# mborhi/CoMA-UNet

Hardware: AMD Instinct MI355X
Metric: volumes/sec (train fwd+bwd) at 128^3 bf16 (higher is better)
Workload: dtype bf16; 1 GPU; CoMA-UNet train step (fwd + RoiMSE/RnC loss + bwd + all-reduce + AdamW), 128^3 volumes, batch 2/GPU, 6-dim covariates (BASELINE configs[3]); global_batch=2, parallelism=dp1, launch=hipGraph replay of the whole step

## Files before the change

### coma_unet_amd/csrc/conv_mfma.hip

```cpp
#include "common.h"
#include <type_traits>

typedef __attribute__((ext_vector_type(8))) short bf16x8_t;
typedef __attribute__((ext_vector_type(16))) float f32x16_t;

template <typename T> struct elem;
template <> struct elem<bf16_t> { static constexpr int EPB = 8; };
template <> struct elem<float> { static constexpr int EPB = 4; };

__device__ __forceinline__ f32x16_t mma_piece(const uint4& a, const uint4& b, f32x16_t acc, bf16_t) {
  return __builtin_amdgcn_mfma_f32_32x32x16_bf16(*reinterpret_cast<const bf16x8_t*>(&a), *reinterpret_cast<const bf16x8_t*>(&b), acc, 0, 0, 0);
}
__device__ __forceinline__ f32x16_t mma_piece(const uint4& a, const uint4& b, f32x16_t acc, float) {
  acc = __builtin_amdgcn_mfma_f32_32x32x2f32(__uint_as_float(a.x), __uint_as_float(b.x), acc, 0, 0, 0);
  acc = __builtin_amdgcn_mfma_f32_32x32x2f32(__uint_as_float(a.y), __uint_as_float(b.y), acc, 0, 0, 0);
  acc = __builtin_amdgcn_mfma_f32_32x32x2f32(__uint_as_float(a.z), __uint_as_float(b.z), acc, 0, 0, 0);
  acc = __builtin_amdgcn_mfma_f32_32x32x2f32(__uint_as_float(a.w), __uint_as_float(b.w), acc, 0, 0, 0);
  return acc;
}

__device__ __forceinline__ void stat_add(double2* rec, int G, int N, int g, int n, double a, double c) {
  const long rs = ((long)G * N * 2 + 7) & ~7L;
  double* q = reinterpret_cast<double*>(rec) + (long)(blockIdx.x & (COMA_STAT_REPLICAS - 1)) * rs + ((long)g * N + n) * 2;
  unsafeAtomicAdd(q, a);
// ... 2896 lines not shown
      if (FORM == 0) acc[t] = __builtin_amdgcn_mfma_f32_32x32x2f32(d, g[t], acc[t], 0, 0, 0);
      else acc[t] = __builtin_amdgcn_mfma_f32_32x32x2f32(g[t], d, acc[t], 0, 0, 0);
    }
  };

  const int npairs = TM >> 1;
  int tile = tile_begin, tix = 0, tiy = 0, tiz = 0;
  while (tile < tile_end && !tile_coords(tile, p.ntx, p.nty, p.ntz, tix, tiy, tiz)) ++tile;
  if (tile < tile_end) load_next(tix << p.lx, tiy << p.ly, tiz << p.lz);
  while (tile < tile_end) {
    int nt = tile + 1, ntix = 0, ntiy = 0, ntiz = 0;
    while (nt < tile_end && !tile_coords(nt, p.ntx, p.nty, p.ntz, ntix, ntiy, ntiz)) ++nt;
    __syncthreads();
    store_tile();
    __syncthreads();
    if (nt < tile_end) load_next(ntix << p.lx, ntiy << p.ly, ntiz << p.lz);
    float dA, dB, gA[NT], gB[NT];
    rd(ps, dA, gA);
    for (int q = ps; q < npairs; q += 2 * ws) {
      rd(q + ws, dB, gB);
      __builtin_amdgcn_sched_barrier(0);
      mm(dA, gA);
      __builtin_amdgcn_sched_barrier(0);
      rd(q + 2 * ws < npairs ? q + 2 * ws : ps, dA, gA);
      __builtin_amdgcn_sched_barrier(0);
      mm(dB, gB);
      __builtin_amdgcn_sched_barrier(0);
    }
    tile = nt; tix = ntix; tiy = ntiy; tiz = ntiz;
  }
  float* wout = p.dwk + (long)b * p.wsb + (long)(blockIdx.x % (unsigned)p.nrep) * p.rep_stride;
  if constexpr (NT == 7) {
    const int c = c0 + fr;
    const bool full = n0 + 32 <= p.N;
#pragma unroll
    for (int t = 0; t < NT; ++t) {
      const int tap = tg + wt * t;
      if (tap < ntaps && c < p.C) {
        float* pe = wout + ((long)tap * p.N + n0 + 4 * fh) * p.C + c;
#pragma unroll
        for (int e = 0; e < 16; ++e) {
          if (full || n0 + (e & 3) + 8 * (e >> 2) + 4 * fh < p.N) {
            if (p.plain) *pe = acc[t][e]; else atomicAdd(pe, acc[t][e]);
          }
          pe += ((e & 3) == 3 ? 5 : 1) * p.C;
        }
      }
    }
  } else {
#pragma unroll
  for (int t = 0; t < NT; ++t) {
#pragma unroll
    for (int e = 0; e < 16; ++e) {
      const int r = (e & 3) + 8 * (e >> 2) + 4 * fh;
      int tap, n, c;
      if (FORM == 0) {
        const int i = tg + wt * t, tp = i * TPT + (fr >> lcp);
        tap = (i < ntiles && tp < ntaps && gch < chg) ? tp : -1; n = n0 + r; c = c0 + gch;
      } else {
        const int i = tg + wt * t, tp = i * TPT + (r >> lcp), nn = r & (CP - 1);
        tap = (i < ntiles && tp < ntaps && nn < chg) ? tp : -1; n = n0 + nn; c = c0 + fr;
      }
      if (tap >= 0 && n < p.N && c < p.C) {
        if (p.plain) wout[((long)tap * p.N + n) * p.C + c] = acc[t][e];
        else atomicAdd(wout + ((long)tap * p.N + n) * p.C + c, acc[t][e]);
      }
    }
  }
  }
}

struct Wgrad2P {
  const bf16_t* dyp; int ldn; long sbn;
  const bf16_t* xp; int ldc; long sbc;
  int N, C, D, H, W;
  int ntx, nty, ntz, tiles_total, tiles_per_block, cblocks;
  int vec_n, vec_c;
  int lgd, lgg;
  float* dwk; long wsb;
  int nrep; long rep_stride;
};

template <int HX, int HY, int NT>
__device__ __forceinline__ void wgrad2_tile(const char* Dt, const char* Gt, int lane_d, int lane_g, const int (&toff)[NT],
                                            int ntap, f32x16_t (&acc)[NT], int ks0, int ksd) {
  constexpr int PD = 64, PG = 64;
  auto rd_d = [&](int ks) -> bf16x8_t {
    const int z = ks >> 3, y = (ks >> 1) & 3, xh = ks & 1;
    const char* dp = Dt + lane_d + ((z * 4 + y) * 32 + xh * 16) * PD;
    const s4_t dlo = __builtin_amdgcn_ds_read_tr16_b64_v4i16((lds_s4_t*)(dp));
    const s4_t dhi = __builtin_amdgcn_ds_read_tr16_b64_v4i16((lds_s4_t*)(dp + 4 * PD));
    return (bf16x8_t){dlo[0], dlo[1], dlo[2], dlo[3], dhi[0], dhi[1], dhi[2], dhi[3]};
  };
  auto rd_g = [&](int ks, int t) -> bf16x8_t {
    const int z = ks >> 3, y = (ks >> 1) & 3, xh = ks & 1;
    const char* gp = Gt + lane_g + ((z * HY + y) * HX + xh * 16) * PG;
    const s4_t glo = __builtin_amdgcn_ds_read_tr16_b64_v4i16((lds_s4_t*)(gp + toff[t]));
    const s4_t ghi = __builtin_amdgcn_ds_read_tr16_b64_v4i16((lds_s4_t*)(gp + toff[t] + 4 * PG));
    return (bf16x8_t){glo[0], glo[1], glo[2], glo[3], ghi[0], ghi[1], ghi[2], ghi[3]};
  };
  (void)ntap;
  bf16x8_t df = rd_d(ks0), gf = rd_g(ks0, 0);
#pragma unroll 2
  for (int ks = ks0; ks < 16; ks += ksd) {
    const int kn = ks + ksd < 16 ? ks + ksd : ks;
    bf16x8_t dn = df;
#pragma unroll
    for (int t = 0; t < NT; ++t) {
      bf16x8_t gn;
      if (t + 1 < NT) gn = rd_g(ks, t + 1);
      else { dn = rd_d(kn); gn = rd_g(kn, 0); }
      __builtin_amdgcn_sched_barrier(0);
      acc[t] = __builtin_amdgcn_mfma_f32_32x32x16_bf16(df, gf, acc[t], 0, 0, 0);
      __builtin_amdgcn_sched_barrier(0);
      gf = gn;
    }
    df = dn;
  }
}

template <int VEC, int OCC, int K, int PK>
__global__ __launch_bounds__(256, OCC) void conv_mfma_wgrad2_k(Wgrad2P p) {
  constexpr int PADK = (K - 1) / 2;
  constexpr int NTILE = K == 1 ? 1 : (PK == 1 ? 27 : PK == 2 ? 18 : 9), NT = (NTILE + 3) / 4;
  constexpr int TX = 32, TY = 4, TZ = 2, TM = TX * TY * TZ, HX = TX + K - 1, HY = TY + K - 1, HZ = TZ + K - 1, HV = HX * HY * HZ;
  constexpr int NDP = TM * 4, NGP = HV * 4;
  constexpr int DIT = NDP / 256, GIT = (NGP + 255) / 256;
  extern __shared__ __attribute__((aligned(16))) char smem[];
  char* Dt = smem;
  char* Gt = smem + TM * 64;
  const int tid = threadIdx.x, lane = tid & 63;
  const int wid = __builtin_amdgcn_readfirstlane(tid >> 6);
  const int b = blockIdx.z;
  const int nb = blockIdx.y / p.cblocks, cb = blockIdx.y % p.cblocks;
  const int n0 = nb * 32, c0 = cb * 32;
  const bf16_t* dyb = p.dyp + (long)b * p.sbn + n0;
  const bf16_t* xb = p.xp + (long)b * p.sbc + c0;
  const int chn = p.N - n0, chc = p.C - c0;
  const int lgd = PK == 1 ? 2 : p.lgd, lgg = PK == 1 ? 2 : p.lgg;
  const int chd = tid & ((1 << lgd) - 1), chg = tid & ((1 << lgg) - 1);
  const bool dlive = chd * 8 < chn, glive = chg * 8 < chc;

  for (int i = tid; i < NDP + NGP; i += 256) reinterpret_cast<uint4*>(smem)[i] = make_uint4(0, 0, 0, 0);

  f32x16_t acc[NT];
#pragma unroll
  for (int t = 0; t < NT; ++t)
#pragma unroll
    for (int e = 0; e < 16; ++e) acc[t][e] = 0.f;

  const int g16 = lane >> 4, li = lane & 15, q = li >> 2, pp = li & 3;
  const int vrow = 8 * (g16 >> 1) + q;
  const int chan_b = ((g16 & 1) * 16 + 4 * pp) * 2;
  const int lane_d = vrow * 64 + chan_b;
  const int chunk = (g16 & 1) * 4 + pp;
  const int lane_g = PK == 1 ? vrow * 64 + chan_b
                   : PK == 2 ? (vrow + (chunk >> 2)) * 64 + (chunk & 3) * 8
                             : (vrow + (chunk >> 1)) * 64 + (chunk & 1) * 8;

  int toff[NT];
#pragma unroll
  for (int t = 0; t < NT; ++t) {
    const int i = wid + 4 * t < NTILE ? wid + 4 * t : 0;
    const int row = PK == 1 ? i / 3 : PK == 2 ? i >> 1 : i, kx0 = PK == 1 ? i % 3 : PK == 2 ? (i & 1) * 2 : 0;
    toff[t] = K == 1 ? 0 : __builtin_amdgcn_readfirstlane((((row / 3) * HY + row % 3) * HX + kx0) * 64);
  }
  const int ntap = K == 1 ? 1 : (NTILE - wid + 3) / 4;

  const int tile_begin = xcd_remap(blockIdx.x, gridDim.x) * p.tiles_per_block;
  int tile_end = tile_begin + p.tiles_per_block;
  if (tile_end > p.tiles_total) tile_end = p.tiles_total;

  uint4 dv[DIT], gv[GIT];
  auto load_tile = [&](int x0, int y0, int z0) {
    if (dlive) {
#pragma unroll
      for (int it = 0; it < DIT; ++it) {
        const int row = (tid + 256 * it) >> lgd;
        const int vx = row & 31, vy = (row >> 5) & 3, vz = row >> 7;
        const int gz = z0 + vz, gy = y0 + vy, gx = x0 + vx;
        dv[it] = make_uint4(0, 0, 0, 0);
        if (row < TM && gz < p.D && gy < p.H && gx < p.W) {
          const bf16_t* src = dyb + (unsigned)(((gz * p.H + gy) * p.W + gx) * p.ldn + chd * 8);
          dv[it] = VEC ? *reinterpret_cast<const uint4*>(src) : load8_raw(src, chn - chd * 8, p.vec_n);
        }
      }
    }
    if (glive) {
#pragma unroll
      for (int it = 0; it < GIT; ++it) {
        const int row = (tid + 256 * it) >> lgg;
        const int hx = row % HX, hy = (row / HX) % HY, hz = row / (HX * HY);
        const int gz = z0 - PADK + hz, gy = y0 - PADK + hy, gx = x0 - PADK + hx;
        gv[it] = make_uint4(0, 0, 0, 0);
        if (row < HV && (unsigned)gz < (unsigned)p.D && (unsigned)gy < (unsigned)p.H && (unsigned)gx < (unsigned)p.W) {
          const bf16_t* src = xb + (unsigned)(((gz * p.H + gy) * p.W + gx) * p.ldc + chg * 8);
          gv[it] = VEC ? *reinterpret_cast<const uint4*>(src) : load8_raw(src, chc - chg * 8, p.vec_c);
        }
      }
    }
  };
  const uint4 dmask = mask8(VEC ? 8 : chn - chd * 8), gmask = mask8(VEC ? 8 : chc - chg * 8);
  auto and4 = [](uint4 v, uint4 m) { v.x &= m.x; v.y &= m.y; v.z &= m.z; v.w &= m.w; return v; };
  auto store_tile = [&]() {
    if (dlive) {
#pragma unroll
      for (int it = 0; it < DIT; ++it) {
        const int row = (tid + 256 * it) >> lgd;
        if (row < TM) reinterpret_cast<uint4*>(Dt)[row * 4 + chd] = VEC ? dv[it] : and4(dv[it], dmask);
      }
    }
    if (glive) {
#pragma unroll
      for (int it = 0; it < GIT; ++it) {
        const int row = (tid + 256 * it) >> lgg;
        if (row < HV) reinterpret_cast<uint4*>(Gt)[row * 4 + chg] = VEC ? gv[it] : and4(gv[it], gmask);
      }
    }
  };

  int tile = tile_begin, tix = 0, tiy = 0, tiz = 0;
  while (tile < tile_end && !tile_coords(tile, p.ntx, p.nty, p.ntz, tix, tiy, tiz)) ++tile;
  if (tile < tile_end) load_tile(tix * TX, tiy * TY, tiz * TZ);
  while (tile < tile_end) {
    int nt = tile + 1, ntix = 0, ntiy = 0, ntiz = 0;
    while (nt < tile_end && !tile_coords(nt, p.ntx, p.nty, p.ntz, ntix, ntiy, ntiz)) ++nt;
    __syncthreads();
    store_tile();
    __syncthreads();
    constexpr bool EARLY = OCC == 1 || PK > 1 || K == 1;
    if (EARLY) { if (nt < tile_end) load_tile(ntix * TX, ntiy * TY, ntiz * TZ); }
    wgrad2_tile<HX, HY, NT>(Dt, Gt, lane_d, lane_g, toff, ntap, acc, K == 1 ? wid : 0, K == 1 ? 4 : 1);
    if (!EARLY) { if (nt < tile_end) load_tile(ntix * TX, ntiy * TY, ntiz * TZ); }
    tile = nt;
  }
  float* wout = p.dwk + (long)b * p.wsb + (long)(blockIdx.x % (unsigned)p.nrep) * p.rep_stride;
  const int fr = lane & 31, fh = lane >> 5;
  const int sub = PK == 1 ? 0 : PK == 2 ? fr >> 4 : fr >> 3;
  const int cc = PK == 1 ? fr : PK == 2 ? (fr & 15) : (fr & 7);
#pragma unroll
  for (int t = 0; t < NT; ++t) {
    const int i = wid + 4 * t;
    const int row = PK == 1 ? i / 3 : PK == 2 ? i >> 1 : i, kx = (PK == 1 ? i % 3 : PK == 2 ? (i & 1) * 2 : 0) + sub;
    const int tap = K == 1 ? 0 : row * 3 + kx;
    if (t < ntap && kx < 3) {
#pragma unroll
      for (int e = 0; e < 16; ++e) {
        const int n = n0 + (e & 3) + 8 * (e >> 2) + 4 * fh;
        const int c = c0 + cc;
        if (n < p.N && c < p.C) atomicAdd(wout + ((long)tap * p.N + n) * p.C + c, acc[t][e]);
      }
    }
  }
}

static bool wgrad2_ok(const coma_conv_desc* d, const coma_tensor* x, const coma_tensor* dy) {
  return d->form == 0 && d->stride == 1 && (d->ksize == 3 || d->ksize == 1) && x->dtype == COMA_BF16 && dy->dtype == COMA_BF16 &&
         x->W >= 32 && (long)t_vox(x) * x->ld < (1L << 31) && (long)t_vox(dy) * dy->ld < (1L << 31);
}

#define WGRAD_NREP 64
#define WGRAD_REP_MAX_ELEMS 16384
static long wgrad_out_elems(const coma_conv_desc* d, const coma_tensor* x, const coma_tensor* dy) {
  return (long)d->ksize * d->ksize * d->ksize * dy->C * x->C * (d->per_sample_w ? x->B : 1);
}
__global__ __launch_bounds__(256) void wgrad_replica_sum_k(const float* __restrict__ rep, int nrep, long n, float* __restrict__ out) {
  const long i = (long)blockIdx.x * 32 + (threadIdx.x >> 3);
  const int part = threadIdx.x & 7;
  float a = 0.f;
  if (i < n) {
#pragma unroll 8
    for (int r = part; r < nrep; r += 8) a += rep[(long)r * n + i];
  }
  a += __shfl_xor(a, 4, 64); a += __shfl_xor(a, 2, 64); a += __shfl_xor(a, 1, 64);
  if (part == 0 && i < n) out[i] = a;
}

struct Thin16FWP {
  const float* x; int ldx; long sbx; int D, H, W, C;
  const float* dy; int ldn; long sbn; int N;
  unsigned xbytes, dbytes;
  int ntx, nty, ntz, ids_total, ids_per_block;
  float* dwk; long wsb;
  int nrep; long rep_stride;
};

template <int CP, int NB>
__global__ __launch_bounds__(256, CP == 16 ? 1 : 2) void conv_thin16f_wgrad_k(Thin16FWP p) {
  constexpr int TX = 32, TY = 4, TZ = 2, HX = TX + 2, HY = TY + 2, HZ = TZ + 2, HV = HX * HY * HZ, TM = TX * TY * TZ;
  constexpr int TPM = 16 / CP, NM = (27 + TPM - 1) / TPM;
  constexpr int ND = NB * 16;
  constexpr int PCH = CP / 4, DCH = ND / 4;
  constexpr int HP = HV * PCH, DP = TM * DCH, HIT = (HP + 255) / 256, DIT = DP / 256, NIT = HIT + DIT;
  static_assert(NIT <= 32, "two staging pieces per K step at most");
  extern __shared__ __attribute__((aligned(16))) char smem[];
  float* Hl = reinterpret_cast<float*>(smem);
  float* Dl = Hl + HV * CP;
  const int tid = threadIdx.x, lane = tid & 63;
  const int wid = __builtin_amdgcn_readfirstlane(tid >> 6);
  const int b = blockIdx.z;
  const int lv = lane & 15, lg = lane >> 4;
  const float* xb = p.x + (long)b * p.sbx;
  const float* db = p.dy + (long)b * p.sbn;
  const __amdgpu_buffer_rsrc_t rs_x = __builtin_amdgcn_make_buffer_rsrc(const_cast<float*>(xb), 0, p.xbytes, 0x00020000);
  const __amdgpu_buffer_rsrc_t rs_d = __builtin_amdgcn_make_buffer_rsrc(const_cast<float*>(db), 0, p.dbytes, 0x00020000);
  constexpr unsigned OOB = 0x7fff0000u;

  int s_z[NIT], s_y[NIT], s_x[NIT];
  unsigned s_boff[NIT];
#pragma unroll
  for (int it = 0; it < NIT; ++it) {
    if (it < HIT) {
      const int piece = tid + 256 * it;
      const int row = piece / PCH, ch = piece % PCH;
      const int hx = row % HX, hy = (row / HX) % HY, hz = row / (HX * HY);
      s_z[it] = piece < HP ? hz - 1 : (1 << 20); s_y[it] = hy - 1; s_x[it] = hx - 1;
      s_boff[it] = (unsigned)(ch * 16);
// ... 666 lines not shown
  q.wsb = d->per_sample_w ? wsz1 : 0;
  q.dwk = dwk;
  if (!(zeroed & COMA_ZEROED_OUT) && hipMemsetAsync(dwk, 0, sizeof(float) * wsz, s) != hipSuccess) { coma_set_error("wgrad memset failed"); return 2; }
  const size_t lds = S == 1 ? (size_t)(34 * 6 * 4 + 256) * 64 : (size_t)(65 * 5 * 3 + 64) * 64;
  static bool attr = false;
  if (!attr) {
    (void)hipFuncSetAttribute((const void*)conv_bf16_wgrad16_k<1, 0>, hipFuncAttributeMaxDynamicSharedMemorySize, 80 * 1024);
    (void)hipFuncSetAttribute((const void*)conv_bf16_wgrad16_k<2, 0>, hipFuncAttributeMaxDynamicSharedMemorySize, 80 * 1024);
    (void)hipFuncSetAttribute((const void*)conv_bf16_wgrad16_k<2, 1>, hipFuncAttributeMaxDynamicSharedMemorySize, 80 * 1024);
    attr = true;
  }
  const dim3 grid((unsigned)gx, (unsigned)pairs, (unsigned)x->B);
  coma_set_kernel_tag("conv_bf16_wgrad16_k<%d, %d>", S, d->form);
  if (S == 1) hipLaunchKernelGGL((conv_bf16_wgrad16_k<1, 0>), grid, dim3(256), lds, s, q);
  else if (d->form == 0) hipLaunchKernelGGL((conv_bf16_wgrad16_k<2, 0>), grid, dim3(256), lds, s, q);
  else hipLaunchKernelGGL((conv_bf16_wgrad16_k<2, 1>), grid, dim3(256), lds, s, q);
  COMA_LAUNCH_CHECK();
  return 0;
}

static bool thin16f_wgrad_ok(const coma_conv_desc* d, const coma_tensor* x, const coma_tensor* dy) {
  static const bool on = []{ const char* e = getenv("COMA_THIN16F"); return !(e && e[0] == '0'); }();
  const int nmax = x->C <= 4 ? 32 : 16;
  return on && d->form == 0 && d->ksize == 3 && d->stride == 1 && x->dtype == COMA_F32 && dy->dtype == COMA_F32 && x->W >= 32 &&
         x->C <= 16 && dy->C <= nmax && x->ld % 4 == 0 && x->sb % 4 == 0 && dy->ld % 4 == 0 && dy->sb % 4 == 0 &&
         (!x->data || aligned16(x->data)) && (!dy->data || aligned16(dy->data)) &&
         (unsigned long long)t_vox(x) * x->ld * 4 < 0x7fff0000ull && (unsigned long long)t_vox(dy) * dy->ld * 4 < 0x7fff0000ull;
}

static int conv_thin16f_wgrad(const coma_conv_desc* d, const coma_tensor* x, const coma_tensor* dy, float* dwk, void* ws,
                              size_t ws_bytes, hipStream_t s, int zeroed) {
  Thin16FWP q;
  q.x = (const float*)x->data; q.ldx = (int)x->ld; q.sbx = x->sb; q.D = x->D; q.H = x->H; q.W = x->W; q.C = x->C;
  q.dy = (const float*)dy->data; q.ldn = (int)dy->ld; q.sbn = dy->sb; q.N = dy->C;
  q.xbytes = (unsigned)((unsigned long long)t_vox(x) * x->ld * 4);
  q.dbytes = (unsigned)((unsigned long long)t_vox(dy) * dy->ld * 4);
  q.ntx = (q.W + 31) / 32; q.nty = (q.H + 3) / 4; q.ntz = (q.D + 1) / 2;
  q.ids_total = q.ntx * q.nty * ((q.ntz + 7) / 8) * 8;
  int gx = (q.C > 8 ? 256 : 512) / x->B;
  if (gx < 1) gx = 1;
  if (gx > q.ids_total) gx = q.ids_total;
  q.ids_per_block = (q.ids_total + gx - 1) / gx;
  gx = (q.ids_total + q.ids_per_block - 1) / q.ids_per_block;
  const long wsz1 = 27L * q.N * q.C, wsz = wsz1 * (d->per_sample_w ? x->B : 1);
  q.wsb = d->per_sample_w ? wsz1 : 0;
  const bool replicas = wsz <= WGRAD_REP_MAX_ELEMS && ws && ws_bytes >= sizeof(float) * wsz * WGRAD_NREP;
  q.nrep = replicas ? WGRAD_NREP : 1;
  q.rep_stride = replicas ? wsz : 0;
  q.dwk = replicas ? (float*)ws : dwk;
  if (!(zeroed & (replicas ? COMA_ZEROED_WS : COMA_ZEROED_OUT)) && hipMemsetAsync(q.dwk, 0, sizeof(float) * wsz * q.nrep, s) != hipSuccess) { coma_set_error("wgrad memset failed"); return 2; }
  const int cp = q.C > 8 ? 16 : q.C > 4 ? 8 : 4, nb = q.N > 16 ? 2 : 1;
  const int nm = (27 + 16 / cp - 1) / (16 / cp);
  size_t lds = (size_t)34 * 6 * 4 * cp * 4 + (size_t)256 * nb * 16 * 4;
  if (lds < (size_t)nm * nb * 256 * 4) lds = (size_t)nm * nb * 256 * 4;
  static bool attr = false;
  if (!attr) {
    (void)hipFuncSetAttribute((const void*)conv_thin16f_wgrad_k<16, 1>, hipFuncAttributeMaxDynamicSharedMemorySize, 80 * 1024);
    (void)hipFuncSetAttribute((const void*)conv_thin16f_wgrad_k<8, 1>, hipFuncAttributeMaxDynamicSharedMemorySize, 80 * 1024);
    (void)hipFuncSetAttribute((const void*)conv_thin16f_wgrad_k<4, 1>, hipFuncAttributeMaxDynamicSharedMemorySize, 80 * 1024);
    (void)hipFuncSetAttribute((const void*)conv_thin16f_wgrad_k<4, 2>, hipFuncAttributeMaxDynamicSharedMemorySize, 80 * 1024);
    attr = true;
  }
  const dim3 grid((unsigned)gx, 1, (unsigned)x->B);
  coma_set_kernel_tag("conv_thin16f_wgrad_k<%d, %d>", cp, nb);
  if (cp == 16) hipLaunchKernelGGL((conv_thin16f_wgrad_k<16, 1>), grid, dim3(256), lds, s, q);
  else if (cp == 8) hipLaunchKernelGGL((conv_thin16f_wgrad_k<8, 1>), grid, dim3(256), lds, s, q);
  else if (nb == 2) hipLaunchKernelGGL((conv_thin16f_wgrad_k<4, 2>), grid, dim3(256), lds, s, q);
  else hipLaunchKernelGGL((conv_thin16f_wgrad_k<4, 1>), grid, dim3(256), lds, s, q);
  COMA_LAUNCH_CHECK();
  if (replicas) {
    hipLaunchKernelGGL(wgrad_replica_sum_k, dim3((unsigned)((wsz + 31) / 32)), dim3(256), 0, s, (const float*)ws, WGRAD_NREP, wsz, dwk);
    COMA_LAUNCH_CHECK();
  }
  return 0;
}

static int conv_mfma_wgrad2(const coma_conv_desc* d, const coma_tensor* x, const coma_tensor* dy, float* dwk, void* ws,
                            size_t ws_bytes, hipStream_t s, int zeroed) {
  Wgrad2P p;
  p.dyp = (const bf16_t*)dy->data; p.ldn = (int)dy->ld; p.sbn = dy->sb;
  p.xp = (const bf16_t*)x->data; p.ldc = (int)x->ld; p.sbc = x->sb;
  p.N = dy->C; p.C = x->C; p.D = x->D; p.H = x->H; p.W = x->W;
  p.ntx = (p.W + 31) / 32; p.nty = (p.H + 3) / 4; p.ntz = (p.D + 1) / 2;
  p.tiles_total = p.ntx * p.nty * ((p.ntz + 7) / 8) * 8;
  p.cblocks = (p.C + 31) / 32;
  {
    const int nd = p.N > 32 ? 4 : (p.N + 7) / 8, ng = p.C > 32 ? 4 : (p.C + 7) / 8;
    p.lgd = nd <= 1 ? 0 : nd <= 2 ? 1 : 2; p.lgg = ng <= 1 ? 0 : ng <= 2 ? 1 : 2;
  }
  const int pairs = ((p.N + 31) / 32) * p.cblocks;
  p.vec_n = dy->ld % 8 == 0 && dy->sb % 8 == 0 && (((uintptr_t)dy->data) & 15) == 0;
  p.vec_c = x->ld % 8 == 0 && x->sb % 8 == 0 && (((uintptr_t)x->data) & 15) == 0;
  int chunks = 512 / (pairs * x->B);
  if (chunks < 1) chunks = 1;
  if (chunks > p.tiles_total) chunks = p.tiles_total;
  p.tiles_per_block = (p.tiles_total + chunks - 1) / chunks;
  chunks = (p.tiles_total + p.tiles_per_block - 1) / p.tiles_per_block;
  const long taps = (long)d->ksize * d->ksize * d->ksize;
  p.dwk = dwk; p.wsb = d->per_sample_w ? taps * p.N * p.C : 0;
  const long wsz = taps * p.N * p.C * (d->per_sample_w ? x->B : 1);
  const bool replicas = wsz <= WGRAD_REP_MAX_ELEMS && ws && ws_bytes >= sizeof(float) * wsz * WGRAD_NREP;
  p.nrep = replicas ? WGRAD_NREP : 1;
  p.rep_stride = replicas ? wsz : 0;
  if (replicas) p.dwk = (float*)ws;
  if (!(zeroed & (replicas ? COMA_ZEROED_WS : COMA_ZEROED_OUT)) && hipMemsetAsync(p.dwk, 0, sizeof(float) * wsz * p.nrep, s) != hipSuccess) { coma_set_error("wgrad memset failed"); return 2; }
  const size_t lds = (size_t)(256 + (d->ksize == 3 ? 816 + 1 : 256)) * 64;
  static bool attr = false;
  if (!attr) {
    (void)hipFuncSetAttribute((const void*)conv_mfma_wgrad2_k<0, 2, 3, 1>, hipFuncAttributeMaxDynamicSharedMemorySize, 80 * 1024);
    (void)hipFuncSetAttribute((const void*)conv_mfma_wgrad2_k<1, 2, 3, 1>, hipFuncAttributeMaxDynamicSharedMemorySize, 80 * 1024);
    (void)hipFuncSetAttribute((const void*)conv_mfma_wgrad2_k<0, 2, 3, 2>, hipFuncAttributeMaxDynamicSharedMemorySize, 80 * 1024);
    (void)hipFuncSetAttribute((const void*)conv_mfma_wgrad2_k<1, 2, 3, 2>, hipFuncAttributeMaxDynamicSharedMemorySize, 80 * 1024);
    (void)hipFuncSetAttribute((const void*)conv_mfma_wgrad2_k<0, 2, 3, 4>, hipFuncAttributeMaxDynamicSharedMemorySize, 80 * 1024);
    (void)hipFuncSetAttribute((const void*)conv_mfma_wgrad2_k<1, 2, 3, 4>, hipFuncAttributeMaxDynamicSharedMemorySize, 80 * 1024);
    attr = true;
  }
  const bool vec = p.vec_n && p.vec_c && p.N % 8 == 0 && p.C % 8 == 0;
  const dim3 grid((unsigned)chunks, (unsigned)pairs, (unsigned)x->B);
  coma_set_kernel_tag("conv_mfma_wgrad2_k<%d, 2, %d, %d>", (int)vec, d->ksize, d->ksize == 1 ? 1 : p.C <= 8 ? 4 : p.C <= 16 ? 2 : 1);
#define WG2(K_, PK_) do { if (vec) hipLaunchKernelGGL((conv_mfma_wgrad2_k<1, 2, K_, PK_>), grid, dim3(256), lds, s, p); \
                          else hipLaunchKernelGGL((conv_mfma_wgrad2_k<0, 2, K_, PK_>), grid, dim3(256), lds, s, p); } while (0)
  if (d->ksize == 1) WG2(1, 1);
  else if (p.C <= 8) WG2(3, 4);
  else if (p.C <= 16) WG2(3, 2);
  else WG2(3, 1);
#undef WG2
  COMA_LAUNCH_CHECK();
  if (replicas) {
    hipLaunchKernelGGL(wgrad_replica_sum_k, dim3((unsigned)((wsz + 31) / 32)), dim3(256), 0, s, (const float*)ws, WGRAD_NREP, wsz, dwk);
    COMA_LAUNCH_CHECK();
  }
  return 0;
}

static int ilog2_ceil(int v) { int l = 0; while ((1 << l) < v) ++l; return l; }

struct WgradPlan { WgradP2 p; int TM; size_t lds; int tn, tc; dim3 grid; bool ok; };

static WgradPlan wgrad_plan(const coma_conv_desc* d, const coma_tensor* x, const coma_tensor* dy) {
  WgradPlan pl{};
  pl.ok = false;
  const bool f32 = x->dtype == COMA_F32 && dy->dtype == COMA_F32;
  if (!f32 && (x->dtype != COMA_BF16 || dy->dtype != COMA_BF16)) return pl;
  if (d->ksize != 3 && d->ksize != 1) return pl;
  if ((long)t_vox(x) * x->ld >= (1L << 31) || (long)t_vox(dy) * dy->ld >= (1L << 31)) return pl;
  if (d->form == 1 && d->stride != 2) return pl;
  WgradP2& p = pl.p;
  p.dyp = dy->data; p.ldn = (int)dy->ld; p.sbn = dy->sb;
  p.xp = x->data; p.ldc = (int)x->ld; p.sbc = x->sb;
  p.N = dy->C; p.C = x->C;
  const coma_tensor* dn = d->form == 0 ? dy : x;
  const coma_tensor* ga = d->form == 0 ? x : dy;
  p.Mz = dn->D; p.My = dn->H; p.Mx = dn->W; p.Gz = ga->D; p.Gy = ga->H; p.Gx = ga->W;
  p.k = d->ksize; p.stride = d->stride; p.pad = d->pad;
  const int vq = f32 ? 4 : 8;
  p.vec_n = dy->ld % vq == 0 && dy->sb % vq == 0 && (!dy->data || aligned16(dy->data));
  p.vec_c = x->ld % vq == 0 && x->sb % vq == 0 && (!x->data || aligned16(x->data));
  pl.tn = (dy->C > 32 && !(x->C > 32 && x->C > dy->C)) ? 2 : 1;
  pl.tc = (pl.tn == 1 && x->C > 32) ? 2 : 1;
  if (f32) pl.tn = pl.tc = 1;
  const int gch = d->form == 0 ? x->C : dy->C;
  const int esz = f32 ? 4 : 2, ppc = f32 ? 4 : 8, maxp = f32 ? ((gch >= 32 && d->ksize == 3) ? 21 : 24) : 20;
  p.cp = 32; p.pg = 128;
  if (f32 && gch < 32) { p.cp = 1; while (p.cp < gch) p.cp <<= 1; p.pg = (p.cp < 4 ? 4 : p.cp) * 4; }
  if (f32 && !(p.vec_n && p.vec_c)) return pl;
  const int cdb = 32 * (d->form == 0 ? pl.tn : pl.tc), cgb = f32 ? p.pg / 4 : 32 * (d->form == 0 ? pl.tc : pl.tn);
  bool fits = false;
  for (int budget = d->stride == 1 ? 8 : 6; budget >= 4 && !fits; --budget) {
    int lx = ilog2_ceil(p.Mx); if (lx > 5) lx = 5;
    if (d->stride == 2 && lx > 4) lx = 4;
    if (lx > budget) lx = budget;
    int rem = budget - lx;
    int ly = ilog2_ceil(p.My); if (ly > (rem + 1) / 2) ly = (rem + 1) / 2;
    rem -= ly;
    int lz = ilog2_ceil(p.Mz); if (lz > rem) lz = rem;
    while (lx + ly + lz < 4) ++lx;
    p.lx = lx; p.ly = ly; p.lz = lz;
    pl.TM = 1 << (lx + ly + lz);
    p.hz = ((1 << lz) - 1) * p.stride + p.k; p.hy = ((1 << ly) - 1) * p.stride + p.k; p.hx = ((1 << lx) - 1) * p.stride + p.k;
    pl.lds = (size_t)pl.TM * cdb * esz + (size_t)p.hz * p.hy * p.hx * cgb * esz + (f32 ? 1024 : 0);
    fits = pl.lds <= 160 * 1024 && pl.TM * (cdb / ppc) + p.hz * p.hy * p.hx * (cgb / ppc) <= 256 * maxp;
  }
  if (!fits) return pl;
  p.ntx = (p.Mx + (1 << p.lx) - 1) >> p.lx; p.nty = (p.My + (1 << p.ly) - 1) >> p.ly; p.ntz = (p.Mz + (1 << p.lz) - 1) >> p.lz;
  p.tiles_total = p.ntx * p.nty * ((p.ntz + 7) / 8) * 8;
  p.m_hx = (unsigned)((1ull << 32) / (unsigned)p.hx) + 1u;
  p.m_hxy = (unsigned)((1ull << 32) / (unsigned)(p.hx * p.hy)) + 1u;
  p.cblocks = (p.C + 32 * pl.tc - 1) / (32 * pl.tc);
  const int pairs = ((p.N + 32 * pl.tn - 1) / (32 * pl.tn)) * p.cblocks;
  int chunks = 256 / (pairs * x->B);
  if (pairs * x->B >= 64 && (long)p.Mz * p.My * p.Mx <= 1024) chunks = 1;
  if (chunks < 1) chunks = 1;
  if (chunks > p.tiles_total) chunks = p.tiles_total;
  p.tiles_per_block = (p.tiles_total + chunks - 1) / chunks;
  chunks = (p.tiles_total + p.tiles_per_block - 1) / p.tiles_per_block;
  p.plain = chunks == 1 && (d->per_sample_w || x->B == 1);
  if (f32 && p.cp < 8 && d->ksize == 3) p.plain = 0;
  if (f32 && d->ksize == 1) p.plain = 0;
  pl.grid = dim3((unsigned)chunks, (unsigned)pairs, (unsigned)x->B);
  const long taps = (long)d->ksize * d->ksize * d->ksize;
  p.wsb = d->per_sample_w ? taps * p.N * p.C : 0;
  pl.ok = true;
  return pl;
}
// ... 76 lines not shown
```

Baseline: 118.7 volumes/s.

## Ping-pong two warp groups in 3x3x3 wgrad kernel to overlap loads with MFMA

For the K=3, PK=1 weight-gradient kernel, the block grows to 512 threads split into two 256-thread groups, each with its own LDS tile buffer. The groups alternate between staging a tile (global load plus LDS store) and computing MFMA on it, synchronized with duo_barrier, so memory traffic of one group overlaps compute of the other. The two groups' partial accumulators are reduced through LDS before the atomic write-out, and the grid halves its chunk count to compensate. The non-group path now always issues the next tile load early. The cost is double LDS per block (up to 160KB), occupancy 1, and an extra cross-group reduction.

After: 119.3 volumes/s, median of 6. About the same (+0.5%).

```diff
diff --git a/coma_unet_amd/csrc/conv_mfma.hip b/coma_unet_amd/csrc/conv_mfma.hip
--- a/coma_unet_amd/csrc/conv_mfma.hip
+++ b/coma_unet_amd/csrc/conv_mfma.hip
@@ -3040,17 +3040,20 @@
 }
 
 template <int VEC, int OCC, int K, int PK>
-__global__ __launch_bounds__(256, OCC) void conv_mfma_wgrad2_k(Wgrad2P p) {
+__global__ __launch_bounds__(K == 3 && PK == 1 ? 512 : 256, K == 3 && PK == 1 ? 1 : OCC) void conv_mfma_wgrad2_k(Wgrad2P p) {
+  constexpr bool GROUPS = K == 3 && PK == 1;
   constexpr int PADK = (K - 1) / 2;
   constexpr int NTILE = K == 1 ? 1 : (PK == 1 ? 27 : PK == 2 ? 18 : 9), NT = (NTILE + 3) / 4;
   constexpr int TX = 32, TY = 4, TZ = 2, TM = TX * TY * TZ, HX = TX + K - 1, HY = TY + K - 1, HZ = TZ + K - 1, HV = HX * HY * HZ;
   constexpr int NDP = TM * 4, NGP = HV * 4;
   constexpr int DIT = NDP / 256, GIT = (NGP + 255) / 256;
+  constexpr int IMG = (TM + HV + 1) * 64;
   extern __shared__ __attribute__((aligned(16))) char smem[];
-  char* Dt = smem;
-  char* Gt = smem + TM * 64;
-  const int tid = threadIdx.x, lane = tid & 63;
-  const int wid = __builtin_amdgcn_readfirstlane(tid >> 6);
+  const int wall = __builtin_amdgcn_readfirstlane(threadIdx.x >> 6);
+  const int grp = GROUPS ? wall >> 2 : 0, wid = wall & 3;
+  const int tid = threadIdx.x & 255, lane = tid & 63;
+  char* Dt = smem + grp * IMG;
+  char* Gt = Dt + TM * 64;
   const int b = blockIdx.z;
   const int nb = blockIdx.y / p.cblocks, cb = blockIdx.y % p.cblocks;
   const int n0 = nb * 32, c0 = cb * 32;
@@ -3061,7 +3064,7 @@
   const int chd = tid & ((1 << lgd) - 1), chg = tid & ((1 << lgg) - 1);
   const bool dlive = chd * 8 < chn, glive = chg * 8 < chc;
 
-  for (int i = tid; i < NDP + NGP; i += 256) reinterpret_cast<uint4*>(smem)[i] = make_uint4(0, 0, 0, 0);
+  for (int i = tid; i < NDP + NGP; i += 256) reinterpret_cast<uint4*>(Dt)[i] = make_uint4(0, 0, 0, 0);
 
   f32x16_t acc[NT];
 #pragma unroll
@@ -3139,6 +3142,60 @@
     }
   };
 
+  if constexpr (GROUPS) {
+    const int nsteps = (tile_end - tile_begin + 1) / 2;
+    auto tile_of = [&](int s, int& x0, int& y0, int& z0) -> bool {
+      const int id = tile_begin + 2 * s + grp;
+      int tx = 0, ty = 0, tz = 0;
+      const bool ok = id < tile_end && tile_coords(id, p.ntx, p.nty, p.ntz, tx, ty, tz);
+      x0 = tx * TX; y0 = ty * TY; z0 = tz * TZ;
+      return __builtin_amdgcn_readfirstlane((int)ok) != 0;
+    };
+    auto stage = [&](int s) __attribute__((always_inline)) {
+      int x0, y0, z0;
+      if (tile_of(s, x0, y0, z0)) { load_tile(x0, y0, z0); store_tile(); }
+    };
+    auto compute = [&](int s) __attribute__((always_inline)) {
+      int x0, y0, z0;
+      if (tile_of(s, x0, y0, z0)) wgrad2_tile<HX, HY, NT>(Dt, Gt, lane_d, lane_g, toff, ntap, acc, 0, 1);
+    };
+    __syncthreads();
+    if (grp == 0) {
+      stage(0);
+      duo_barrier();
+#pragma unroll 1
+      for (int s = 0; s < nsteps; ++s) {
+        compute(s); duo_barrier();
+        stage(s + 1); duo_barrier();
+      }
+    } else {
+      duo_barrier();
+#pragma unroll 1
+      for (int s = 0; s < nsteps; ++s) {
+        stage(s); duo_barrier();
+        compute(s); duo_barrier();
+      }
+    }
+    __syncthreads();
+    f32x4_t* xa = reinterpret_cast<f32x4_t*>(smem) + wid * (NT * 4 * 64) + lane;
+    if (grp == 1) {
+#pragma unroll
+      for (int t = 0; t < NT; ++t)
+#pragma unroll
+        for (int j = 0; j < 4; ++j)
+          xa[(t * 4 + j) * 64] = (f32x4_t){acc[t][4 * j], acc[t][4 * j + 1], acc[t][4 * j + 2], acc[t][4 * j + 3]};
+    }
+    __syncthreads();
+    if (grp == 1) return;
+#pragma unroll
+    for (int t = 0; t < NT; ++t)
+#pragma unroll
+      for (int j = 0; j < 4; ++j) {
+        const f32x4_t v = xa[(t * 4 + j) * 64];
+#pragma unroll
+        for (int e = 0; e < 4; ++e) acc[t][4 * j + e] += v[e];
+      }
+  } else {
   int tile = tile_begin, tix = 0, tiy = 0, tiz = 0;
   while (tile < tile_end && !tile_coords(tile, p.ntx, p.nty, p.ntz, tix, tiy, tiz)) ++tile;
   if (tile < tile_end) load_tile(tix * TX, tiy * TY, tiz * TZ);
@@ -3148,11 +3205,10 @@
     __syncthreads();
     store_tile();
     __syncthreads();
-    constexpr bool EARLY = OCC == 1 || PK > 1 || K == 1;
-    if (EARLY) { if (nt < tile_end) load_tile(ntix * TX, ntiy * TY, ntiz * TZ); }
+    if (nt < tile_end) load_tile(ntix * TX, ntiy * TY, ntiz * TZ);
     wgrad2_tile<HX, HY, NT>(Dt, Gt, lane_d, lane_g, toff, ntap, acc, K == 1 ? wid : 0, K == 1 ? 4 : 1);
-    if (!EARLY) { if (nt < tile_end) load_tile(ntix * TX, ntiy * TY, ntiz * TZ); }
     tile = nt;
+  }
   }
   float* wout = p.dwk + (long)b * p.wsb + (long)(blockIdx.x % (unsigned)p.nrep) * p.rep_stride;
   const int fr = lane & 31, fh = lane >> 5;
@@ -3994,7 +4050,8 @@
   const int pairs = ((p.N + 31) / 32) * p.cblocks;
   p.vec_n = dy->ld % 8 == 0 && dy->sb % 8 == 0 && (((uintptr_t)dy->data) & 15) == 0;
   p.vec_c = x->ld % 8 == 0 && x->sb % 8 == 0 && (((uintptr_t)x->data) & 15) == 0;
-  int chunks = 512 / (pairs * x->B);
+  const bool groups = d->ksize == 3 && p.C > 16;
+  int chunks = (groups ? 256 : 512) / (pairs * x->B);
   if (chunks < 1) chunks = 1;
   if (chunks > p.tiles_total) chunks = p.tiles_total;
   p.tiles_per_block = (p.tiles_total + chunks - 1) / chunks;
@@ -4007,11 +4064,11 @@
   p.rep_stride = replicas ? wsz : 0;
   if (replicas) p.dwk = (float*)ws;
   if (!(zeroed & (replicas ? COMA_ZEROED_WS : COMA_ZEROED_OUT)) && hipMemsetAsync(p.dwk, 0, sizeof(float) * wsz * p.nrep, s) != hipSuccess) { coma_set_error("wgrad memset failed"); return 2; }
-  const size_t lds = (size_t)(256 + (d->ksize == 3 ? 816 + 1 : 256)) * 64;
+  const size_t lds = (size_t)(256 + (d->ksize == 3 ? 816 + 1 : 256)) * 64 * (groups ? 2 : 1);
   static bool attr = false;
   if (!attr) {
-    (void)hipFuncSetAttribute((const void*)conv_mfma_wgrad2_k<0, 2, 3, 1>, hipFuncAttributeMaxDynamicSharedMemorySize, 80 * 1024);
-    (void)hipFuncSetAttribute((const void*)conv_mfma_wgrad2_k<1, 2, 3, 1>, hipFuncAttributeMaxDynamicSharedMemorySize, 80 * 1024);
+    (void)hipFuncSetAttribute((const void*)conv_mfma_wgrad2_k<0, 2, 3, 1>, hipFuncAttributeMaxDynamicSharedMemorySize, 160 * 1024);
+    (void)hipFuncSetAttribute((const void*)conv_mfma_wgrad2_k<1, 2, 3, 1>, hipFuncAttributeMaxDynamicSharedMemorySize, 160 * 1024);
     (void)hipFuncSetAttribute((const void*)conv_mfma_wgrad2_k<0, 2, 3, 2>, hipFuncAttributeMaxDynamicSharedMemorySize, 80 * 1024);
     (void)hipFuncSetAttribute((const void*)conv_mfma_wgrad2_k<1, 2, 3, 2>, hipFuncAttributeMaxDynamicSharedMemorySize, 80 * 1024);
     (void)hipFuncSetAttribute((const void*)conv_mfma_wgrad2_k<0, 2, 3, 4>, hipFuncAttributeMaxDynamicSharedMemorySize, 80 * 1024);
@@ -4021,8 +4078,9 @@
   const bool vec = p.vec_n && p.vec_c && p.N % 8 == 0 && p.C % 8 == 0;
   const dim3 grid((unsigned)chunks, (unsigned)pairs, (unsigned)x->B);
   coma_set_kernel_tag("conv_mfma_wgrad2_k<%d, 2, %d, %d>", (int)vec, d->ksize, d->ksize == 1 ? 1 : p.C <= 8 ? 4 : p.C <= 16 ? 2 : 1);
-#define WG2(K_, PK_) do { if (vec) hipLaunchKernelGGL((conv_mfma_wgrad2_k<1, 2, K_, PK_>), grid, dim3(256), lds, s, p); \
-                          else hipLaunchKernelGGL((conv_mfma_wgrad2_k<0, 2, K_, PK_>), grid, dim3(256), lds, s, p); } while (0)
+  const dim3 block(groups ? 512 : 256);
+#define WG2(K_, PK_) do { if (vec) hipLaunchKernelGGL((conv_mfma_wgrad2_k<1, 2, K_, PK_>), grid, block, lds, s, p); \
+                          else hipLaunchKernelGGL((conv_mfma_wgrad2_k<0, 2, K_, PK_>), grid, block, lds, s, p); } while (0)
   if (d->ksize == 1) WG2(1, 1);
   else if (p.C <= 8) WG2(3, 4);
   else if (p.C <= 16) WG2(3, 2);
```

## Reuse halo z-planes across consecutive tiles in 3x3x3 wgrad via LDS ring

Applied to the files above, without the earlier changes.

For 3x3x3 weight-gradient convolutions, tiles are now walked z-first within each (x,y) column, and the input halo is kept in a 4-plane LDS ring. Each new tile loads only the TZ new z-planes instead of the full HZ-plane halo, and only the first tile of a column loads the full halo. Per-tap LDS offsets are recomputed each tile from the ring position. This cuts global input traffic and LDS stores, but makes tile ordering column-major, so load-balancing and the locality of blocks across XCDs change. The early/late prefetch choice is also removed, so the next tile is always prefetched before compute.

After: 118.7 volumes/s before, 119.4 volumes/s after, median of 6. No clear change (+0.6%).

```diff
diff --git a/coma_unet_amd/csrc/conv_mfma.hip b/coma_unet_amd/csrc/conv_mfma.hip
--- a/coma_unet_amd/csrc/conv_mfma.hip
+++ b/coma_unet_amd/csrc/conv_mfma.hip
@@ -3002,8 +3002,8 @@
 };
 
 template <int HX, int HY, int NT>
-__device__ __forceinline__ void wgrad2_tile(const char* Dt, const char* Gt, int lane_d, int lane_g, const int (&toff)[NT],
-                                            int ntap, f32x16_t (&acc)[NT], int ks0, int ksd) {
+__device__ __forceinline__ void wgrad2_tile(const char* Dt, const char* Gt, int lane_d, int lane_g, const int (&toff0)[NT],
+                                            const int (&toff1)[NT], int ntap, f32x16_t (&acc)[NT], int ks0, int ksd) {
   constexpr int PD = 64, PG = 64;
   auto rd_d = [&](int ks) -> bf16x8_t {
     const int z = ks >> 3, y = (ks >> 1) & 3, xh = ks & 1;
@@ -3015,8 +3015,9 @@
   auto rd_g = [&](int ks, int t) -> bf16x8_t {
     const int z = ks >> 3, y = (ks >> 1) & 3, xh = ks & 1;
     const char* gp = Gt + lane_g + ((z * HY + y) * HX + xh * 16) * PG;
-    const s4_t glo = __builtin_amdgcn_ds_read_tr16_b64_v4i16((lds_s4_t*)(gp + toff[t]));
-    const s4_t ghi = __builtin_amdgcn_ds_read_tr16_b64_v4i16((lds_s4_t*)(gp + toff[t] + 4 * PG));
+    const int to = z ? toff1[t] : toff0[t];
+    const s4_t glo = __builtin_amdgcn_ds_read_tr16_b64_v4i16((lds_s4_t*)(gp + to));
+    const s4_t ghi = __builtin_amdgcn_ds_read_tr16_b64_v4i16((lds_s4_t*)(gp + to + 4 * PG));
     return (bf16x8_t){glo[0], glo[1], glo[2], glo[3], ghi[0], ghi[1], ghi[2], ghi[3]};
   };
   (void)ntap;
@@ -3039,12 +3040,23 @@
   }
 }
 
+__device__ __forceinline__ bool wgrad2_tile_coords(int id, int nty, int ntz, int& tix, int& tiy, int& tiz) {
+  const int col = id / ntz;
+  tiz = id - col * ntz;
+  tix = col / nty;
+  tiy = col - tix * nty;
+  return true;
+}
+
 template <int VEC, int OCC, int K, int PK>
 __global__ __launch_bounds__(256, OCC) void conv_mfma_wgrad2_k(Wgrad2P p) {
   constexpr int PADK = (K - 1) / 2;
   constexpr int NTILE = K == 1 ? 1 : (PK == 1 ? 27 : PK == 2 ? 18 : 9), NT = (NTILE + 3) / 4;
   constexpr int TX = 32, TY = 4, TZ = 2, TM = TX * TY * TZ, HX = TX + K - 1, HY = TY + K - 1, HZ = TZ + K - 1, HV = HX * HY * HZ;
-  constexpr int NDP = TM * 4, NGP = HV * 4;
+  constexpr bool RING = K == 3;
+  constexpr int PLR = HX * HY, PLB = PLR * 64;
+  constexpr int GROWS = RING ? TZ * PLR : HV;
+  constexpr int NDP = TM * 4, NGP = GROWS * 4;
   constexpr int DIT = NDP / 256, GIT = (NGP + 255) / 256;
   extern __shared__ __attribute__((aligned(16))) char smem[];
   char* Dt = smem;
@@ -3061,7 +3073,7 @@
   const int chd = tid & ((1 << lgd) - 1), chg = tid & ((1 << lgg) - 1);
   const bool dlive = chd * 8 < chn, glive = chg * 8 < chc;
 
-  for (int i = tid; i < NDP + NGP; i += 256) reinterpret_cast<uint4*>(smem)[i] = make_uint4(0, 0, 0, 0);
+  for (int i = tid; i < (TM + HV) * 4; i += 256) reinterpret_cast<uint4*>(smem)[i] = make_uint4(0, 0, 0, 0);
 
   f32x16_t acc[NT];
 #pragma unroll
@@ -3078,21 +3090,25 @@
                    : PK == 2 ? (vrow + (chunk >> 2)) * 64 + (chunk & 3) * 8
                              : (vrow + (chunk >> 1)) * 64 + (chunk & 1) * 8;
 
-  int toff[NT];
+  int tkz[NT], trow[NT];
 #pragma unroll
   for (int t = 0; t < NT; ++t) {
     const int i = wid + 4 * t < NTILE ? wid + 4 * t : 0;
     const int row = PK == 1 ? i / 3 : PK == 2 ? i >> 1 : i, kx0 = PK == 1 ? i % 3 : PK == 2 ? (i & 1) * 2 : 0;
-    toff[t] = K == 1 ? 0 : __builtin_amdgcn_readfirstlane((((row / 3) * HY + row % 3) * HX + kx0) * 64);
+    tkz[t] = K == 1 ? 0 : row / 3;
+    trow[t] = K == 1 ? 0 : ((row % 3) * HX + kx0) * 64;
   }
   const int ntap = K == 1 ? 1 : (NTILE - wid + 3) / 4;
 
   const int tile_begin = xcd_remap(blockIdx.x, gridDim.x) * p.tiles_per_block;
   int tile_end = tile_begin + p.tiles_per_block;
   if (tile_end > p.tiles_total) tile_end = p.tiles_total;
+  auto coords = [&](int id, int& tix, int& tiy, int& tiz) {
+    return RING ? wgrad2_tile_coords(id, p.nty, p.ntz, tix, tiy, tiz) : tile_coords(id, p.ntx, p.nty, p.ntz, tix, tiy, tiz);
+  };
 
   uint4 dv[DIT], gv[GIT];
-  auto load_tile = [&](int x0, int y0, int z0) {
+  auto load_d = [&](int x0, int y0, int z0) __attribute__((always_inline)) {
     if (dlive) {
 #pragma unroll
       for (int it = 0; it < DIT; ++it) {
@@ -3106,14 +3122,16 @@
         }
       }
     }
+  };
+  auto load_g = [&](int x0, int y0, int zp) __attribute__((always_inline)) {
     if (glive) {
 #pragma unroll
       for (int it = 0; it < GIT; ++it) {
         const int row = (tid + 256 * it) >> lgg;
         const int hx = row % HX, hy = (row / HX) % HY, hz = row / (HX * HY);
-        const int gz = z0 - PADK + hz, gy = y0 - PADK + hy, gx = x0 - PADK + hx;
+        const int gz = zp + hz, gy = y0 - PADK + hy, gx = x0 - PADK + hx;
         gv[it] = make_uint4(0, 0, 0, 0);
-        if (row < HV && (unsigned)gz < (unsigned)p.D && (unsigned)gy < (unsigned)p.H && (unsigned)gx < (unsigned)p.W) {
+        if (row < GROWS && (unsigned)gz < (unsigned)p.D && (unsigned)gy < (unsigned)p.H && (unsigned)gx < (unsigned)p.W) {
           const bf16_t* src = xb + (unsigned)(((gz * p.H + gy) * p.W + gx) * p.ldc + chg * 8);
           gv[it] = VEC ? *reinterpret_cast<const uint4*>(src) : load8_raw(src, chc - chg * 8, p.vec_c);
         }
@@ -3122,7 +3140,7 @@
   };
   const uint4 dmask = mask8(VEC ? 8 : chn - chd * 8), gmask = mask8(VEC ? 8 : chc - chg * 8);
   auto and4 = [](uint4 v, uint4 m) { v.x &= m.x; v.y &= m.y; v.z &= m.z; v.w &= m.w; return v; };
-  auto store_tile = [&]() {
+  auto store_d = [&]() __attribute__((always_inline)) {
     if (dlive) {
 #pragma unroll
       for (int it = 0; it < DIT; ++it) {
@@ -3130,29 +3148,52 @@
         if (row < TM) reinterpret_cast<uint4*>(Dt)[row * 4 + chd] = VEC ? dv[it] : and4(dv[it], dmask);
       }
     }
+  };
+  auto store_g = [&](int slot) __attribute__((always_inline)) {
     if (glive) {
+      uint4* dst = reinterpret_cast<uint4*>(Gt + slot * PLB);
 #pragma unroll
       for (int it = 0; it < GIT; ++it) {
         const int row = (tid + 256 * it) >> lgg;
-        if (row < HV) reinterpret_cast<uint4*>(Gt)[row * 4 + chg] = VEC ? gv[it] : and4(gv[it], gmask);
-      }
-    }
-  };
-
-  int tile = tile_begin, tix = 0, tiy = 0, tiz = 0;
-  while (tile < tile_end && !tile_coords(tile, p.ntx, p.nty, p.ntz, tix, tiy, tiz)) ++tile;
-  if (tile < tile_end) load_tile(tix * TX, tiy * TY, tiz * TZ);
+        if (row < GROWS) dst[row * 4 + chg] = VEC ? gv[it] : and4(gv[it], gmask);
+      }
+    }
+  };
+  auto load_tile = [&](int tx, int ty, int tz) __attribute__((always_inline)) {
+    load_d(tx * TX, ty * TY, tz * TZ);
+    load_g(tx * TX, ty * TY, tz * TZ - PADK + (RING ? TZ : 0));
+  };
+
+  int tile = tile_begin, tix = 0, tiy = 0, tiz = 0, ring = 0;
+  bool fresh = true;
+  while (tile < tile_end && !coords(tile, tix, tiy, tiz)) ++tile;
+  if (tile < tile_end) load_tile(tix, tiy, tiz);
   while (tile < tile_end) {
     int nt = tile + 1, ntix = 0, ntiy = 0, ntiz = 0;
-    while (nt < tile_end && !tile_coords(nt, p.ntx, p.nty, p.ntz, ntix, ntiy, ntiz)) ++nt;
+    while (nt < tile_end && !coords(nt, ntix, ntiy, ntiz)) ++nt;
     __syncthreads();
-    store_tile();
+    store_d();
+    if (RING) {
+      ring = fresh ? 0 : ring ^ 2;
+      store_g(ring ^ 2);
+      if (fresh) {
+        load_g(tix * TX, tiy * TY, tiz * TZ - PADK);
+        store_g(0);
+      }
+    } else {
+      store_g(0);
+    }
     __syncthreads();
-    constexpr bool EARLY = OCC == 1 || PK > 1 || K == 1;
-    if (EARLY) { if (nt < tile_end) load_tile(ntix * TX, ntiy * TY, ntiz * TZ); }
-    wgrad2_tile<HX, HY, NT>(Dt, Gt, lane_d, lane_g, toff, ntap, acc, K == 1 ? wid : 0, K == 1 ? 4 : 1);
-    if (!EARLY) { if (nt < tile_end) load_tile(ntix * TX, ntiy * TY, ntiz * TZ); }
-    tile = nt;
+    int toff0[NT], toff1[NT];
+#pragma unroll
+    for (int t = 0; t < NT; ++t) {
+      toff0[t] = RING ? __builtin_amdgcn_readfirstlane(((ring + tkz[t]) & 3) * PLB + trow[t]) : 0;
+      toff1[t] = RING ? __builtin_amdgcn_readfirstlane((((ring + 1 + tkz[t]) & 3) - 1) * PLB + trow[t]) : 0;
+    }
+    if (nt < tile_end) load_tile(ntix, ntiy, ntiz);
+    wgrad2_tile<HX, HY, NT>(Dt, Gt, lane_d, lane_g, toff0, toff1, ntap, acc, K == 1 ? wid : 0, K == 1 ? 4 : 1);
+    fresh = ntiz == 0;
+    tile = nt; tix = ntix; tiy = ntiy; tiz = ntiz;
   }
   float* wout = p.dwk + (long)b * p.wsb + (long)(blockIdx.x % (unsigned)p.nrep) * p.rep_stride;
   const int fr = lane & 31, fh = lane >> 5;
@@ -3985,7 +4026,7 @@
   p.xp = (const bf16_t*)x->data; p.ldc = (int)x->ld; p.sbc = x->sb;
   p.N = dy->C; p.C = x->C; p.D = x->D; p.H = x->H; p.W = x->W;
   p.ntx = (p.W + 31) / 32; p.nty = (p.H + 3) / 4; p.ntz = (p.D + 1) / 2;
-  p.tiles_total = p.ntx * p.nty * ((p.ntz + 7) / 8) * 8;
+  p.tiles_total = d->ksize == 3 ? p.ntx * p.nty * p.ntz : p.ntx * p.nty * ((p.ntz + 7) / 8) * 8;
   p.cblocks = (p.C + 31) / 32;
   {
     const int nd = p.N > 32 ? 4 : (p.N + 7) / 8, ng = p.C > 32 ? 4 : (p.C + 7) / 8;
```
